# baaivision/Painter

Hardware: AMD Instinct MI355X
Metric: images/sec (896x448 pairs) ViT-L fwd+bwd (higher is better)
Workload: dtype bf16; 1 GPU; painter_vit_large_patch16_input896x448 bf16 batch=8/GPU fwd+bwd on 1xMI355X (BASELINE configs[1]); global_batch=8, image=896x448x3 stitched pair, mode=train (DropPath 0.1), parallelism=dp1, rccl_ranks=0, backend=n/a, grad_allreduce=n/a

## Files before the change

### include/painter_hip.h

```cpp
#ifndef PAINTER_HIP_H
#define PAINTER_HIP_H

#include <stdint.h>

#ifdef __cplusplus
extern "C" {
#endif

#ifndef __HIP__
typedef struct ihipStream_t* hipStream_t;
#endif

enum { PA_F32 = 0, PA_BF16 = 1 };
enum {
    PA_EPI_BIAS = 0,
    PA_EPI_BIAS_F32 = 1,
    PA_EPI_BIAS_GELU = 2,
    PA_EPI_BIAS_RESID = 3
};

#define PA_ABI_VERSION 9
int pa_abi_version(void);
int pa_debug_set(int which, int value);
int pa_debug_get(int which);
// ... 102 lines not shown
int pa_cast_bf16(const float* in, void* out, int64_t n, hipStream_t stream);
int pa_debug_rmw(const float* src, float* scratch, int64_t n, int passes, int nblocks, hipStream_t stream);
int pa_ensemble_resid(const float* x0, const float* a, float* x1, int batch, int group, int L, int D, hipStream_t stream);

int pa_conv3x3_pack(int dtype, const float* w3 , void* w3r , void* wf ,
                    hipStream_t stream);
int pa_decoder_tail_fwd(int dtype, const void* x_nhwc, const void* w3r, const float* b3, const float* ln_gamma,
                        const float* ln_beta, const float* w1 , const float* b1, void* y3 ,
                        float* pred , int batch, int Hi, int Wi, float eps, hipStream_t stream);
int64_t pa_decoder_tail_bwd_workspace_bytes(int batch, int Hi, int Wi);
int pa_decoder_tail_bwd_pointwise(int dtype, const float* dpred, const void* y3, const float* ln_gamma,
                                  const float* ln_beta, const float* w1, void* dy3, float* grads, void* workspace,
                                  int batch, int Hi, int Wi, float eps, hipStream_t stream);
int pa_conv3x3_dgrad_unshuffle(int dtype, const void* dy3, const void* wf, void* dE, int batch, int Hp, int Wp, int P,
                               hipStream_t stream);
int64_t pa_conv3x3_wgrad_workspace_bytes(int batch, int Hi, int Wi);
int pa_conv3x3_wgrad(int dtype, const void* dy3, const void* x_nhwc, float* dw , void* workspace,
                     int batch, int Hi, int Wi, hipStream_t stream);

int pa_live_rows_max(void);
int pa_live_rows(const unsigned char* mask, int mask_batch_stride, int* rowmap, int* live, int* count, int batch, int Hp, int Wp,
                 hipStream_t stream);
int pa_conv3x3_dgrad_unshuffle_live(const void* dy3, const void* wf, void* dE_compact, const int* rowmap, const int* count, int batch,
                                    int Hp, int Wp, int P, hipStream_t stream);
int pa_gather_rows(const void* src, int64_t src_row_bytes, void* dst, int64_t dst_row_bytes, int64_t row_bytes, const int* live,
                   const int* count, int M, hipStream_t stream);
int pa_linear_dgrad_live(const void* dy, int64_t lddy, const void* w, void* dx, int64_t lddx, const int* live, const int* rowmap,
                         const int* count, int M, int N, int K, hipStream_t stream);
int pa_linear_wgrad_live(const void* dy, int64_t lddy, const void* x, int64_t ldx, float* dw, const int* count, int M, int N, int K,
                         hipStream_t stream);
int pa_colsum_live(int dtype, const void* x, int64_t ld, int M, int N, float* out, void* workspace, const int* count, hipStream_t stream);
int pa_fill_dead_rows(void* x, int64_t pitch_bytes, int64_t row_bytes, const int* rowmap, int M, hipStream_t stream);
int pa_decoder_live_ok(int dtype, int batch, int Hp, int Wp, int P, int Kin);

int64_t pa_loss_workspace_bytes(int batch, int Hi, int Wi);
int pa_loss_fwd(const float* pred, const float* tgts, float* valid, const unsigned char* mask, int mask_batch_stride,
                float* out, void* workspace, int batch, int Hi, int Wi, int P, int ignore_rule, float eps_den, int kind,
                float beta, hipStream_t stream);
int pa_loss_bwd(const float* pred, const float* tgts, const float* valid, const unsigned char* mask,
                int mask_batch_stride, const float* dloss, const float* loss_out, float* dpred, int batch, int Hi, int Wi,
                int P, int kind, float beta, hipStream_t stream);
int pa_patchify(const float* img, float* out, int batch, int Hp, int Wp, int P, hipStream_t stream);
int pa_pred_bwd(const float* pred, const float* tgts, const float* valid, const unsigned char* mask, int mask_batch_stride,
                const float* dloss, const float* loss_out, const float* dpatch, float* dpred, float* dpred_loss, int batch, int Hi,
                int Wi, int P, int kind, float beta, hipStream_t stream);

typedef struct PaOptTensor {
    void* p; const void* g; void* m; void* v;
    void* w16;
    int64_t n;
    int32_t group;
    int32_t first_chunk;
} PaOptTensor;
typedef struct PaOptGroups {
    float lr[64], wd[64];
} PaOptGroups;
int pa_opt_chunk_elems(void);
int64_t pa_grad_sumsq_workspace_bytes(int nchunks);
int pa_grad_sumsq(const PaOptTensor* table, int ntensors, int nchunks, float* out2, void* workspace, hipStream_t stream);
int pa_adamw_step(const PaOptTensor* table, int ntensors, int nchunks, const PaOptGroups* groups, double beta1, double beta2,
                  float eps, float* steps, const float* norm_info, const float* grad_scale, const float* found_inf,
                  float max_norm, hipStream_t stream);

int pa_resample_u8(const void* src, int src_h, int src_w, void* dst, int dst_h, int dst_w, int channels, const void* bounds,
                   const void* coeffs, int ksize, int vertical, hipStream_t stream);
int pa_gather_u8(const void* src, int src_h, int src_w, void* dst, int dst_h, int dst_w, int channels, const void* ytab,
// ... 150 lines not shown
```

### painter_amd/csrc/common.h

```cpp
#pragma once
#include <hip/hip_runtime.h>
#include <stdint.h>
#include <cstdlib>

typedef __bf16 bf16;
typedef __attribute__((ext_vector_type(8))) __bf16 bf16x8;
typedef __attribute__((ext_vector_type(16))) float f32x16;

#define DEVI __device__ __forceinline__

template <typename T> struct TT;
template <> struct TT<float> {
    static constexpr int EPC = 4;
    static constexpr int BK = 32;
    static constexpr int KSTEPS = 2;
    static constexpr int SPF = 2;
    typedef uint4 Vec4;
};
template <> struct TT<bf16> {
    static constexpr int EPC = 8;
    static constexpr int BK = 64;
    static constexpr int KSTEPS = 4;
    static constexpr int SPF = 1;
    typedef uint2 Vec4;
// ... 67 lines not shown
    return v;
}

enum Knob {
    KNOB_G256_STAGGER = 0,
    KNOB_G256_NOSTORE = 1,
    KNOB_G256_ORDER = 2,
    KNOB_WGRAD_TARGET = 3,
    KNOB_G256_SHORT_TILES = 4,
    KNOB_G256_ILV = 5,
    KNOB_RELPOS_SPLITS = 6,
    KNOB_ATTN3_FUSE = 7,
    KNOB_ATTN_LIGHT_LAST = 8,
    KNOB_CONV_WGRAD_GROUPS = 9,
    KNOB_LN_BWD_VARIANT = 10,
    KNOB_G256_PATCH = 11,
    KNOB_G256_MIXED = 12,
    KNOB_FREE_13 = 13,
    KNOB_G256_MIXED_NFULL = 14,
    KNOB_FREE_15 = 15,
    KNOB_DROP_SKIP = 16,
    KNOB_DECODER_ROWS = 17,
    KNOB_COUNT = 18
};
inline int g_knob[KNOB_COUNT] = {};
static inline bool drop_skip_on() {
    static const int env = [] { const char* v = getenv("PAINTER_AMD_DROP_SKIP"); return v ? atoi(v) : 1; }();
    return g_knob[KNOB_DROP_SKIP] == 1 ? false : (g_knob[KNOB_DROP_SKIP] == 2 ? true : env != 0);
}
static inline bool decoder_rows_on() {
    static const int env = [] { const char* v = getenv("PAINTER_AMD_DECODER_ROWS"); return v ? atoi(v) : 1; }();
    return g_knob[KNOB_DECODER_ROWS] == 1 ? false : (g_knob[KNOB_DECODER_ROWS] == 2 ? true : env != 0);
}

inline long long g_attn_counts[6] = {0, 0, 0, 0, 0, 0};

DEVI float gelu_f(float x) { return 0.5f * x * (1.0f + erff(x * 0.70710678118654752f)); }
DEVI float gelu_grad_f(float x) {
    const float cdf = 0.5f * (1.0f + erff(x * 0.70710678118654752f));
    const float pdf = 0.39894228040143268f * __expf(-0.5f * x * x);
    return cdf + x * pdf;
}

DEVI void gelu_parts(float x, float& cdf, float& pdf_unnorm) {
    const float z = fabsf(x) * 0.70710678118654752f;
    const float t = __builtin_amdgcn_rcpf(fmaf(0.3275911f, z, 1.0f));
    const float e = __builtin_amdgcn_exp2f(-0.72134752044448170f * x * x);
    float p = fmaf(1.061405429f, t, -1.453152027f);
    p = fmaf(p, t, 1.421413741f);
    p = fmaf(p, t, -0.284496736f);
    p = fmaf(p, t, 0.254829592f);
    const float half_erfc = 0.5f * p * t * e;
    cdf = x >= 0.f ? 1.0f - half_erfc : half_erfc;
    pdf_unnorm = e;
}
DEVI float gelu_fast(float x) {
    float c, e;
    gelu_parts(x, c, e);
    return x * c;
}
typedef __attribute__((ext_vector_type(2))) float f32x2_t;
DEVI void gelu_parts2(f32x2_t x, f32x2_t& cdf, f32x2_t& e) {
    const f32x2_t ax = {fabsf(x[0]), fabsf(x[1])};
    const f32x2_t d = __builtin_elementwise_fma(ax, (f32x2_t){0.23164189f, 0.23164189f}, (f32x2_t){1.0f, 1.0f});
    const f32x2_t t = {__builtin_amdgcn_rcpf(d[0]), __builtin_amdgcn_rcpf(d[1])};
    const f32x2_t xx = x * x * (f32x2_t){-0.72134752044448170f, -0.72134752044448170f};
// ... 53 lines not shown
```

### painter_amd/csrc/elementwise.hip

```cpp
#include "common.h"
#include "../../include/painter_hip.h"

extern "C" int pa_slab_reduce(const float* in, float* out, int64_t n, int nz, int64_t stride, int accumulate, hipStream_t st);

__global__ void cast_bf16_kernel(const float* __restrict__ in, bf16* __restrict__ out, size_t n) {
    size_t i = ((size_t)blockIdx.x * blockDim.x + threadIdx.x) * 4;
    if (i + 4 <= n) {
        const float4 v = *reinterpret_cast<const float4*>(in + i);
        *reinterpret_cast<uint2*>(out + i) = make_uint2(pack_bf16x2(v.x, v.y), pack_bf16x2(v.z, v.w));
    } else {
        for (; i < n; ++i) out[i] = (bf16)in[i];
    }
}
extern "C" int pa_cast_bf16(const float* in, void* out, int64_t n, hipStream_t st) {
    if (n <= 0) return 0;
    PA_LAUNCH(cast_bf16_kernel, dim3((unsigned)((n + 1023) / 1024)), dim3(256), 0, st, in, (bf16*)out, (size_t)n);
    LAUNCH_CHECK();
}

__global__ __launch_bounds__(256) void sparse_rows_kernel(const int* __restrict__ idx, const float* __restrict__ val, int K, const float* __restrict__ x0,
                                                          const float* __restrict__ x1, float* __restrict__ out, int D) {
    __shared__ float red[4][64];
    const int r = blockIdx.y, cl = threadIdx.x & 63, jl = threadIdx.x >> 6, n = blockIdx.x * 64 + cl;
    float acc = 0.f;
// ... 283 lines not shown
        g += dpatch[((size_t)b * L + l) * (size_t)(3 * P * P) + k];
    }
    dpred[idx] = g;
}
extern "C" int pa_pred_bwd(const float* pred, const float* tgts, const float* valid, const unsigned char* mask, int mask_batch_stride,
                           const float* dloss, const float* loss_out, const float* dpatch, float* dpred, float* dpred_loss, int batch, int Hi,
                           int Wi, int P, int kind, float beta, hipStream_t st) {
    if ((dloss == nullptr && dpatch == nullptr) || (dpred_loss != nullptr && dloss == nullptr) || P < 1 || Hi % P || Wi % P)
        return (int)hipErrorInvalidValue;
    const int HW = Hi * Wi;
    PA_LAUNCH(pred_bwd_kernel, dim3((3 * HW + 255) / 256, batch), dim3(256), 0, st, pred, tgts, valid, mask, mask_batch_stride,
              dloss, loss_out, dpatch, dpred, dpred_loss, HW, Wi, P, Wi / P, kind, beta);
    LAUNCH_CHECK();
}

__global__ void patchify_kernel(const float* __restrict__ img, float* __restrict__ out, int Hp, int Wp, int P, size_t n) {
    const size_t i = (size_t)blockIdx.x * blockDim.x + threadIdx.x;
    if (i >= n) return;
    const int PP3 = P * P * 3, L = Hp * Wp;
    const int k = (int)(i % PP3);
    const size_t t = i / PP3;
    const int l = (int)(t % L), b = (int)(t / L);
    const int c = k % 3, q = (k / 3) % P, p = k / (3 * P), h = l / Wp, w = l % Wp;
    out[i] = img[(((size_t)b * 3 + c) * Hp * P + h * P + p) * (size_t)(Wp * P) + w * P + q];
}
extern "C" int pa_patchify(const float* img, float* out, int batch, int Hp, int Wp, int P, hipStream_t st) {
    const size_t n = (size_t)batch * Hp * Wp * P * P * 3;
    PA_LAUNCH(patchify_kernel, dim3((unsigned)((n + 255) / 256)), dim3(256), 0, st, img, out, Hp, Wp, P, n);
    LAUNCH_CHECK();
}

#define TAILP 324
DEVI float oct_sum(float v) { v = quad_sum(v); v += lane_dpp<0x141>(v); return v; }
template <typename T>
__global__ __launch_bounds__(256) void tail_bwd_kernel(const float* __restrict__ dpred, const T* __restrict__ y3, const float* __restrict__ gamma,
                                                       const float* __restrict__ beta, const float* __restrict__ w1, T* __restrict__ dy3,
                                                       float* __restrict__ part, int HW, int npix, float eps) {
    const int lane = threadIdx.x & 63, wave = threadIdx.x >> 6;
    const int sub = lane & 7, slot = (threadIdx.x >> 3);
    const int c0 = sub * 8;
    f32x2_t g2[4], b2[4], w2[3][4];
#pragma unroll
    for (int k = 0; k < 4; ++k) {
        g2[k] = (f32x2_t){gamma[c0 + 2 * k], gamma[c0 + 2 * k + 1]};
        b2[k] = (f32x2_t){beta[c0 + 2 * k], beta[c0 + 2 * k + 1]};
#pragma unroll
        for (int o = 0; o < 3; ++o) w2[o][k] = (f32x2_t){w1[o * 64 + c0 + 2 * k], w1[o * 64 + c0 + 2 * k + 1]};
    }
    const f32x2_t zero2 = {0.f, 0.f};
    f32x2_t ag[4] = {zero2, zero2, zero2, zero2}, ab[4] = {zero2, zero2, zero2, zero2};
    f32x2_t aw[3][4] = {{zero2, zero2, zero2, zero2}, {zero2, zero2, zero2, zero2}, {zero2, zero2, zero2, zero2}};
    float ab1[3] = {0.f, 0.f, 0.f};
    const int stride = gridDim.x * 32;
    struct In { uint4 a, b; float d0, d1, d2; };
    struct Pos { int pix, b, rem; };
    auto advance = [&](Pos& p) {
        p.pix += stride;
        p.rem += stride;
        while (p.rem >= HW) { p.rem -= HW; ++p.b; }
    };
    auto fetch = [&](const Pos& p) {
        In in;
        const int q = min(p.pix, npix - 1);
        const int bb = p.pix < npix ? p.b : (npix - 1) / HW, rr = p.pix < npix ? p.rem : (npix - 1) % HW;
        in.a = *reinterpret_cast<const uint4*>(y3 + (size_t)q * 64 + c0);
        if constexpr (sizeof(T) == 4) in.b = *reinterpret_cast<const uint4*>(y3 + (size_t)q * 64 + c0 + 4);
        else in.b = in.a;
        const float* dp = dpred + (size_t)bb * 3 * HW + rr;
        in.d0 = dp[0]; in.d1 = dp[(size_t)HW]; in.d2 = dp[(size_t)2 * HW];
        return in;
    };
    Pos cur, nxt;
    cur.pix = blockIdx.x * 32 + slot;
    cur.b = cur.pix / HW;
    cur.rem = cur.pix - cur.b * HW;
    nxt = cur;
    In in0 = fetch(nxt);
    advance(nxt);
    In in1 = fetch(nxt);
    advance(nxt);
    for (; cur.pix < npix; advance(cur)) {
        const In in = in0;
        in0 = in1;
        in1 = fetch(nxt);
        advance(nxt);
        const int pix = cur.pix;
        f32x2_t y[4];
        if constexpr (sizeof(T) == 2) {
            const uint4 raw = in.a;
            y[0] = (f32x2_t){bf16_lo(raw.x), bf16_hi(raw.x)}; y[1] = (f32x2_t){bf16_lo(raw.y), bf16_hi(raw.y)};
            y[2] = (f32x2_t){bf16_lo(raw.z), bf16_hi(raw.z)}; y[3] = (f32x2_t){bf16_lo(raw.w), bf16_hi(raw.w)};
        } else {
            y[0] = (f32x2_t){__builtin_bit_cast(float, in.a.x), __builtin_bit_cast(float, in.a.y)};
            y[1] = (f32x2_t){__builtin_bit_cast(float, in.a.z), __builtin_bit_cast(float, in.a.w)};
            y[2] = (f32x2_t){__builtin_bit_cast(float, in.b.x), __builtin_bit_cast(float, in.b.y)};
            y[3] = (f32x2_t){__builtin_bit_cast(float, in.b.z), __builtin_bit_cast(float, in.b.w)};
        }
        const float d0 = in.d0, d1 = in.d1, d2 = in.d2;
        f32x2_t s2 = (y[0] + y[1]) + (y[2] + y[3]);
        const float mu = oct_sum(s2[0] + s2[1]) * (1.f / 64);
        const f32x2_t mu2 = {mu, mu};
        f32x2_t q2 = zero2;
#pragma unroll
        for (int k = 0; k < 4; ++k) { y[k] = y[k] - mu2; q2 = __builtin_elementwise_fma(y[k], y[k], q2); }
        const float rs = 1.f / sqrtf(oct_sum(q2[0] + q2[1]) * (1.f / 64) + eps);
        const f32x2_t rs2 = {rs, rs}, dd0 = {d0, d0}, dd1 = {d1, d1}, dd2 = {d2, d2};
        f32x2_t dxh[4], m1 = zero2, m2 = zero2;
#pragma unroll
        for (int k = 0; k < 4; ++k) {
            const f32x2_t xh = y[k] * rs2;
            const f32x2_t z = __builtin_elementwise_fma(xh, g2[k], b2[k]);
            f32x2_t a, gz;
            if constexpr (sizeof(T) == 2) {
                gelu_both2(z[0], z[1], a, gz);
            } else {
                a = (f32x2_t){gelu_f(z[0]), gelu_f(z[1])};
                gz = (f32x2_t){gelu_grad_f(z[0]), gelu_grad_f(z[1])};
            }
            const f32x2_t da = __builtin_elementwise_fma(dd2, w2[2][k], __builtin_elementwise_fma(dd1, w2[1][k], dd0 * w2[0][k]));
            const f32x2_t dz = da * gz;
            ag[k] = __builtin_elementwise_fma(dz, xh, ag[k]);
            ab[k] = ab[k] + dz;
            aw[0][k] = __builtin_elementwise_fma(dd0, a, aw[0][k]);
            aw[1][k] = __builtin_elementwise_fma(dd1, a, aw[1][k]);
            aw[2][k] = __builtin_elementwise_fma(dd2, a, aw[2][k]);
            dxh[k] = dz * g2[k];
            m1 = m1 + dxh[k];
            m2 = __builtin_elementwise_fma(dxh[k], xh, m2);
            y[k] = xh;
        }
        if (sub == 0) { ab1[0] += d0; ab1[1] += d1; ab1[2] += d2; }
        const float m1s = oct_sum(m1[0] + m1[1]) * (1.f / 64), m2s = oct_sum(m2[0] + m2[1]) * (1.f / 64);
        const f32x2_t mm1 = {m1s, m1s}, nm2 = {-m2s, -m2s};
        f32x2_t r[4];
#pragma unroll
        for (int k = 0; k < 4; ++k) r[k] = rs2 * (__builtin_elementwise_fma(y[k], nm2, dxh[k]) - mm1);
        if constexpr (sizeof(T) == 2) {
            *reinterpret_cast<uint4*>(dy3 + (size_t)pix * 64 + c0) = make_uint4(pack_bf16x2(r[0][0], r[0][1]), pack_bf16x2(r[1][0], r[1][1]),
                                                                                 pack_bf16x2(r[2][0], r[2][1]), pack_bf16x2(r[3][0], r[3][1]));
        } else {
            *reinterpret_cast<float4*>(dy3 + (size_t)pix * 64 + c0) = make_float4(r[0][0], r[0][1], r[1][0], r[1][1]);
            *reinterpret_cast<float4*>(dy3 + (size_t)pix * 64 + c0 + 4) = make_float4(r[2][0], r[2][1], r[3][0], r[3][1]);
        }
    }
    auto wsum = [&](float v) { v += lane_dpp<0x128>(v); v += lane_xor16(v); v += lane_xor32(v); return v; };
    __shared__ float red[4][TAILP];
#pragma unroll
    for (int k = 0; k < 4; ++k)
#pragma unroll
        for (int e = 0; e < 2; ++e) {
            const float vg = wsum(ag[k][e]), vb = wsum(ab[k][e]), v0 = wsum(aw[0][k][e]), v1 = wsum(aw[1][k][e]), v2 = wsum(aw[2][k][e]);
            if (lane < 8) {
                const int c = c0 + 2 * k + e;
                red[wave][c] = vg; red[wave][64 + c] = vb; red[wave][128 + c] = v0; red[wave][192 + c] = v1; red[wave][256 + c] = v2;
            }
        }
    {
        const float t0 = wsum(ab1[0]), t1 = wsum(ab1[1]), t2 = wsum(ab1[2]);
        if (lane == 0) { red[wave][320] = t0; red[wave][321] = t1; red[wave][322] = t2; red[wave][323] = 0.f; }
    }
    __syncthreads();
    for (int i = threadIdx.x; i < TAILP; i += 256) part[(size_t)blockIdx.x * TAILP + i] = (red[0][i] + red[1][i]) + (red[2][i] + red[3][i]);
}
static int tail_bwd_blocks(int npix) {
    int b = (npix + 31) / 32;
    return b > 2048 ? 2048 : b;
}
extern "C" int64_t pa_decoder_tail_bwd_workspace_bytes(int batch, int Hi, int Wi) { return (int64_t)tail_bwd_blocks(batch * Hi * Wi) * TAILP * sizeof(float); }
extern "C" int pa_decoder_tail_bwd_pointwise(int dtype, const float* dpred, const void* y3, const float* ln_gamma, const float* ln_beta,
                                             const float* w1, void* dy3, float* grads, void* workspace, int batch, int Hi, int Wi, float eps,
                                             hipStream_t st) {
    const int npix = batch * Hi * Wi, nb = tail_bwd_blocks(npix);
    float* part = reinterpret_cast<float*>(workspace);
    if (dtype == PA_BF16)
        PA_LAUNCH(tail_bwd_kernel<bf16>, dim3(nb), dim3(256), 0, st, dpred, (const bf16*)y3, ln_gamma, ln_beta, w1, (bf16*)dy3, part, Hi * Wi, npix, eps);
    else
        PA_LAUNCH(tail_bwd_kernel<float>, dim3(nb), dim3(256), 0, st, dpred, (const float*)y3, ln_gamma, ln_beta, w1, (float*)dy3, part, Hi * Wi, npix, eps);
    int e = (int)hipGetLastError();
    if (e) return e;
    return pa_slab_reduce(part, grads, TAILP, nb, TAILP, 0, st);
}

#define LIVE_NT 1024
#define LIVE_MAX_ROWS 49152
__global__ __launch_bounds__(LIVE_NT) void live_rows_kernel(const unsigned char* __restrict__ mask, int mbs, int* __restrict__ rowmap, int* __restrict__ live,
                                                            int* __restrict__ count, int Bn, int Hp, int Wp) {
    __shared__ int sc[2][LIVE_NT];
    extern __shared__ unsigned char flag[];
    const int L = Hp * Wp, n = Bn * L, per = (n + LIVE_NT - 1) / LIVE_NT;
    for (int t = threadIdx.x; t < n; t += LIVE_NT) {
        const int b = t / L, l = t - b * L, i = l / Wp, j = l - i * Wp;
        const unsigned char* m = mask + (size_t)b * mbs;
        unsigned int any = 0;
#pragma unroll
        for (int di = -1; di <= 1; ++di)
#pragma unroll
            for (int dj = -1; dj <= 1; ++dj) {
                const int ii = i + di, jj = j + dj;
                const bool in = ii >= 0 && ii < Hp && jj >= 0 && jj < Wp;
                any |= in ? (unsigned int)m[in ? ii * Wp + jj : 0] : 0u;
            }
        flag[t] = any ? 1 : 0;
    }
    __syncthreads();
    const int t0 = min(n, (int)threadIdx.x * per), t1 = min(n, t0 + per);
    int mine = 0;
    for (int t = t0; t < t1; ++t) mine += flag[t];
    sc[0][threadIdx.x] = mine;
    __syncthreads();
    int cur = 0;
    for (int d = 1; d < LIVE_NT; d <<= 1) {
        const int v = sc[cur][threadIdx.x] + ((int)threadIdx.x >= d ? sc[cur][threadIdx.x - d] : 0);
        sc[cur ^ 1][threadIdx.x] = v;
        cur ^= 1;
        __syncthreads();
    }
    int at = sc[cur][threadIdx.x] - mine;
    for (int t = t0; t < t1; ++t) {
        if (flag[t]) { rowmap[t] = at; live[at] = t; ++at; }
        else rowmap[t] = -1;
    }
    if (threadIdx.x == LIVE_NT - 1) count[0] = sc[cur][LIVE_NT - 1];
}
extern "C" int pa_live_rows_max(void) { return LIVE_MAX_ROWS; }
extern "C" int pa_live_rows(const unsigned char* mask, int mask_batch_stride, int* rowmap, int* live, int* count, int batch, int Hp, int Wp,
                            hipStream_t st) {
    if (batch < 1 || Hp < 1 || Wp < 1 || (int64_t)batch * Hp * Wp > LIVE_MAX_ROWS) return (int)hipErrorInvalidValue;
    const int n = batch * Hp * Wp;
    PA_LAUNCH(live_rows_kernel, dim3(1), dim3(LIVE_NT), (size_t)((n + 15) & ~15), st, mask, mask_batch_stride, rowmap, live, count, batch, Hp, Wp);
    LAUNCH_CHECK();
}
__global__ __launch_bounds__(256) void gather_rows_kernel(const uint4* __restrict__ src, size_t lds16, uint4* __restrict__ dst, size_t ldd16, int row16,
                                                          const int* __restrict__ live, const int* __restrict__ count) {
    const int r = blockIdx.x, cnt = *count;
    if (r >= ((cnt + 127) & ~127)) return;
    if (r < cnt && src == nullptr) return;
    const uint4* s = r < cnt ? src + (size_t)live[r] * lds16 : nullptr;
    uint4* d = dst + (size_t)r * ldd16;
    for (int c = threadIdx.x; c < row16; c += 256) d[c] = s ? s[c] : zero4();
}
extern "C" int pa_gather_rows(const void* src, int64_t src_row_bytes, void* dst, int64_t dst_row_bytes, int64_t row_bytes, const int* live,
                              const int* count, int M, hipStream_t st) {
    if (M < 1 || row_bytes % 16 || src_row_bytes % 16 || dst_row_bytes % 16 || row_bytes > dst_row_bytes || (src != nullptr && row_bytes > src_row_bytes))
        return (int)hipErrorInvalidValue;
    if (((uintptr_t)src | (uintptr_t)dst) & 15) return (int)hipErrorInvalidValue;
    const int Mp = (M + 127) / 128 * 128;
    PA_LAUNCH(gather_rows_kernel, dim3(Mp), dim3(256), 0, st, (const uint4*)src, (size_t)(src_row_bytes / 16), (uint4*)dst, (size_t)(dst_row_bytes / 16),
              (int)(row_bytes / 16), live, count);
    LAUNCH_CHECK();
}
__global__ __launch_bounds__(256) void fill_dead_rows_kernel(uint4* __restrict__ x, size_t pitch16, size_t row16, const int* __restrict__ rowmap) {
    const int r = blockIdx.x;
    if (rowmap[r] >= 0) return;
    uint4* d = x + (size_t)r * pitch16;
    for (size_t c = threadIdx.x; c < row16; c += 256) d[c] = zero4();
}
extern "C" int pa_fill_dead_rows(void* x, int64_t pitch_bytes, int64_t row_bytes, const int* rowmap, int M, hipStream_t st) {
    if (M < 1 || row_bytes % 16 || pitch_bytes % 16 || row_bytes > pitch_bytes || ((uintptr_t)x & 15)) return (int)hipErrorInvalidValue;
    PA_LAUNCH(fill_dead_rows_kernel, dim3(M), dim3(256), 0, st, (uint4*)x, (size_t)(pitch_bytes / 16), (size_t)(row_bytes / 16), rowmap);
    LAUNCH_CHECK();
}

__global__ __launch_bounds__(256) void debug_rmw_kernel(const float* __restrict__ src, float* __restrict__ scratch, size_t n4, int passes) {
    for (int p = 0; p < passes; ++p)
// ... 13 lines not shown
```

### painter_amd/engine.py

```python
import os
from typing import NamedTuple

import torch

from . import hostmath, ops
from ._lib import EPI_BIAS, EPI_BIAS_F32, EPI_BIAS_RESID, KNOB_RELPOS_SPLITS, KNOB_WGRAD_TARGET


_SIDE_STREAM = os.environ.get("PAINTER_AMD_SIDE_STREAM", "1") != "0"
_DBG_SERIAL = os.environ.get("PAINTER_AMD_DEBUG_SERIAL", "0") == "1"
_DBG_TRACE = os.environ.get("PAINTER_AMD_DEBUG_TRACE", "0") == "1"
_configured = False
WGRAD_SIDE_TARGET = 96
RELPOS_SIDE_SPLITS = 8


def _configure_library():
    global _configured
    if _configured:
        return
    from ._lib import lib
    lib.pa_debug_set(KNOB_RELPOS_SPLITS, RELPOS_SIDE_SPLITS if _SIDE_STREAM else 0)
    lib.pa_debug_set(KNOB_WGRAD_TARGET, WGRAD_SIDE_TARGET if _SIDE_STREAM else 0)
    _configured = True
# ... 350 lines not shown
        self.trace = []
        dconcat, dpred_loss = self._backward_decoder(X, dloss, dpatch, want_tgts)
        dx = dyT_next = None
        for i in reversed(range(self.cfg.depth)):
            dx, dyT_next = self._backward_block(X, i, dconcat, dx, dyT_next)
        dimgs, dtgts = self._backward_tokens(X, dx, dpred_loss, want_imgs, want_tgts)
        del dpred_loss
        G = X.G
        if want is not None:
            G = {n: g for n, g in G.items() if g is not None and n in want}
        X.st.join(getattr(self, "tail_probe", None))
        if sync is not None:
            sync.finish()
        if want_imgs or want_tgts:
            return G, dimgs, dtgts
        return G

    def _tr(self, name, t):
        if _DBG_TRACE:
            self.trace.append((name, t.detach().double().abs().sum()))

    def _backward_decoder(self, X, dloss, dpatch, want_tgts):
        c, T, P, S, G, st, need = self.cfg, self.T, X.P, X.S, X.G, X.st, X.need
        B = S.B
        dpred_loss = None
        if dpatch is None:
            dpred = ops.loss_bwd(S.pred, S.tgts, S.valid, S.mask, dloss, S.loss_out, c.P, c.loss_func)
            if want_tgts:
                dpred_loss = dpred
        else:
            dpred, dpred_loss = ops.pred_bwd(S.pred, S.tgts, S.valid, S.mask, dloss, S.loss_out, dpatch, c.P, c.loss_func,
                                             want_loss_term=want_tgts and dloss is not None)
        w1 = P["decoder_pred.3.weight"].reshape(3, c.dec)
        dy3, tg = ops.decoder_tail_bwd_pointwise(dpred, S.y3, P["decoder_pred.1.weight"], P["decoder_pred.1.bias"], w1, 1e-6)
        G["decoder_pred.1.weight"] = tg[0:64]
        G["decoder_pred.1.bias"] = tg[64:128]
        G["decoder_pred.3.weight"] = tg[128:320].reshape(3, c.dec, 1, 1)
        G["decoder_pred.3.bias"] = tg[320:323]
        npix = B * c.H * c.W
        if need("decoder_pred.0.weight") or need("decoder_pred.0.bias"):
            G["decoder_pred.0.weight"], G["decoder_pred.0.bias"] = st.run(
                lambda: (ops.conv3x3_wgrad(dy3, S.E) if need("decoder_pred.0.weight") else None,
                         ops.colsum(dy3.view(npix, c.dec)) if need("decoder_pred.0.bias") else None), dy3, S.E)
        w_de = self.w("decoder_embed.weight", P)
        if dpatch is None and ops.decoder_live_ok(T, B, c.Hp, c.Wp, c.P, w_de.shape[1]):
            rowmap, live, count = ops.live_rows(S.mask, B, c.Hp, c.Wp)
            st.shared(count)
            dE = ops.conv3x3_dgrad_unshuffle_live(dy3, S.wf, rowmap, count, B, c.Hp, c.Wp, c.P)
            del dy3
            X.param_grads("decoder_embed.weight", "decoder_embed.bias", dE, S.concat,
                          wgrad=lambda dy, x: ops.linear_wgrad(dy, x, live=(live, count)),
                          colsum=lambda dy, out=None: ops.colsum_live(dy, count, out=out))
            dconcat = ops.linear_dgrad(dE, w_de, live=(live, rowmap, count))
            if _DBG_TRACE:
                self._tr("dE", dE[:int(count.item())])
        else:
            dE = ops.conv3x3_dgrad_unshuffle(dy3, S.wf, B, c.Hp, c.Wp, c.P)
            del dy3
            X.param_grads("decoder_embed.weight", "decoder_embed.bias", dE, S.concat)
            dconcat = ops.linear_dgrad(dE, w_de)
            self._tr("dE", dE)
        self._tr("dconcat", dconcat)
        del dE
        X.ready(["decoder_embed.weight", "decoder_embed.bias"])
        X.ready([n for n in G if n.startswith("decoder_pred.")])
        return dconcat, dpred_loss

    def block_flat(self, X, i):
        if i not in X.flats:
            D = self.cfg.D
            sizes = [2 * D, 2 * D, 3 * D, D, self.cfg.hidden, D, X.rc_shape[0] * X.rc_shape[1]]
            fb = X.st.shared(torch.empty((sum(sizes),), dtype=torch.float32, device=X.S.imgs.device))
            X.flats[i] = (fb, dict(zip(("n1", "n2", "qkv", "proj", "fc1", "fc2", "rel"), torch.split(fb, sizes))))
        return X.flats[i]

    def _backward_block(self, X, i, dconcat, dx, dyT_next):
        c, T, P, S, G, st, need = self.cfg, self.T, X.P, X.S, X.G, X.st, X.need
        B, L, D = S.B, c.L, c.D
        dev = S.imgs.device
# ... 131 lines not shown
```

### painter_amd/ops.py

```python
import torch

from ._lib import (EPI_BIAS, EPI_BIAS_F32, EPI_BIAS_GELU, EPI_BIAS_RESID, KNOB_DECODER_ROWS, KNOB_DROP_SKIP, PA_BF16, PA_F32, check, lib)

_WS = {}


def stream():
    return torch.cuda.current_stream().cuda_stream


def code(dtype):
    if dtype == torch.bfloat16:
        return PA_BF16
    if dtype == torch.float32:
        return PA_F32
    raise TypeError("painter_amd supports float32 / bfloat16 operand types, got %s" % dtype)


def p(t):
    return 0 if t is None else t.data_ptr()


def workspace(nbytes, device, slot=0):
    key = (device, slot, torch.cuda.current_stream(device).cuda_stream)
# ... 126 lines not shown
    if out is None:
        out = torch.empty((N, K), dtype=torch.float32, device=dy.device)
    ws = workspace(lib.pa_linear_wgrad_workspace_bytes(code(T), M, N, K), dy.device)
    check(lib.pa_linear_wgrad(code(T), p(dy), dy.stride(0), p(x), x.stride(0), p(out), p(ws), M, N, K, stream()),
          "pa_linear_wgrad")
    return out


def colsum(x, out=None):
    M, N = x.shape
    if out is None:
        out = torch.empty((N,), dtype=torch.float32, device=x.device)
    ws = workspace(lib.pa_colsum_workspace_bytes(M, N), x.device)
    check(lib.pa_colsum(code(x.dtype), p(x), x.stride(0), M, N, p(out), p(ws), stream()), "pa_colsum")
    return out


def decoder_rows(mode=None):
    return _knob(KNOB_DECODER_ROWS, mode)


def decoder_live_ok(T, batch, Hp, Wp, P, Kin):
    return T == torch.bfloat16 and bool(lib.pa_decoder_live_ok(code(T), batch, Hp, Wp, P, Kin))


def live_rows(mask_u8, batch, Hp, Wp):
    n = batch * Hp * Wp
    assert mask_u8.dtype in (torch.uint8, torch.bool) and mask_u8.is_cuda and mask_u8.stride(-1) == 1 and mask_u8.shape[-1] == Hp * Wp
    assert mask_u8.shape[0] in (1, batch)
    buf = torch.empty((2 * n + 1,), dtype=torch.int32, device=mask_u8.device)
    rowmap, live, count = buf[:n], buf[n:2 * n], buf[2 * n:]
    check(lib.pa_live_rows(p(mask_u8), _mbs(mask_u8), p(rowmap), p(live), p(count), batch, Hp, Wp, stream()), "pa_live_rows")
    return rowmap, live, count


def padded_rows(n):
    return (n + 127) // 128 * 128


def conv3x3_dgrad_unshuffle_live(dy3, wf, rowmap, count, batch, Hp, Wp, P, out=None):
    assert dy3.dtype == torch.bfloat16
    if out is None:
        out = torch.empty((padded_rows(batch * Hp * Wp), P * P * 64), dtype=dy3.dtype, device=dy3.device)
    assert out.shape == (padded_rows(batch * Hp * Wp), P * P * 64) and out.is_contiguous()
    check(lib.pa_conv3x3_dgrad_unshuffle_live(p(dy3), p(wf), p(out), p(rowmap), p(count), batch, Hp, Wp, P, stream()),
          "pa_conv3x3_dgrad_unshuffle_live")
    return out


def gather_rows(x, live, count, out=None):
    M, N = x.shape
    _req(x)
    if out is None:
        out = torch.empty((padded_rows(M), N), dtype=x.dtype, device=x.device)
    es = x.element_size()
    check(lib.pa_gather_rows(p(x), x.stride(0) * es, p(out), out.stride(0) * es, N * es, p(live), p(count), M, stream()), "pa_gather_rows")
    return out


def linear_wgrad_live(dy, x, count, out=None):
    M, N = dy.shape
    K = x.shape[1]
    _req(dy, torch.bfloat16); _req(x, torch.bfloat16)
    assert x.shape[0] == M and M % 128 == 0
    if out is None:
        out = torch.empty((N, K), dtype=torch.float32, device=dy.device)
# ... 269 lines not shown
    x1 = torch.empty_like(x0)
    check(lib.pa_ensemble_resid(p(x0), p(a), p(x1), batch, group, L, D, stream()), "pa_ensemble_resid")
    return x1


def conv3x3_pack(w3, T):
    w3r = torch.empty((64, 9, 64), dtype=T, device=w3.device)
    wf = torch.empty((64, 9, 64), dtype=T, device=w3.device)
    check(lib.pa_conv3x3_pack(code(T), p(w3), p(w3r), p(wf), stream()), "pa_conv3x3_pack")
    return w3r, wf


def decoder_tail_fwd(x_nhwc, w3r, b3, gamma, beta, w1, b1, eps, save_y3=True):
    B, Hi, Wi, C = x_nhwc.shape
    T = x_nhwc.dtype
    y3 = torch.empty((B, Hi, Wi, C), dtype=T, device=x_nhwc.device) if save_y3 else None
    pred = torch.empty((B, 3, Hi, Wi), dtype=torch.float32, device=x_nhwc.device)
    check(lib.pa_decoder_tail_fwd(code(T), p(x_nhwc), p(w3r), p(b3), p(gamma), p(beta), p(w1), p(b1), p(y3), p(pred), B, Hi, Wi,
                                  float(eps), stream()), "pa_decoder_tail_fwd")
    return pred, y3


def decoder_tail_bwd_pointwise(dpred, y3, gamma, beta, w1, eps):
    B, Hi, Wi, C = y3.shape
    T = y3.dtype
    dy3 = torch.empty_like(y3)
    grads = torch.empty((324,), dtype=torch.float32, device=y3.device)
    ws = workspace(lib.pa_decoder_tail_bwd_workspace_bytes(B, Hi, Wi), y3.device)
    check(lib.pa_decoder_tail_bwd_pointwise(code(T), p(dpred), p(y3), p(gamma), p(beta), p(w1), p(dy3), p(grads), p(ws), B, Hi, Wi,
                                            float(eps), stream()), "pa_decoder_tail_bwd_pointwise")
    return dy3, grads


def conv3x3_dgrad_unshuffle(dy3, wf, batch, Hp, Wp, P):
    T = dy3.dtype
    dE = torch.empty((batch * Hp * Wp, P * P * 64), dtype=T, device=dy3.device)
    check(lib.pa_conv3x3_dgrad_unshuffle(code(T), p(dy3), p(wf), p(dE), batch, Hp, Wp, P, stream()), "pa_conv3x3_dgrad_unshuffle")
    return dE


def conv3x3_wgrad(dy3, x_nhwc):
    B, Hi, Wi, C = x_nhwc.shape
    dw = torch.empty((64, 64, 3, 3), dtype=torch.float32, device=dy3.device)
    ws = workspace(lib.pa_conv3x3_wgrad_workspace_bytes(B, Hi, Wi), dy3.device)
    check(lib.pa_conv3x3_wgrad(code(dy3.dtype), p(dy3), p(x_nhwc), p(dw), p(ws), B, Hi, Wi, stream()), "pa_conv3x3_wgrad")
    return dw


LOSS_KINDS = {"smoothl1": 0, "l1": 1, "l2": 2, "l1l2": 3}


def loss_fwd(pred, tgts, valid, mask_u8, P, ignore_rule, eps_den, kind, beta=0.01):
    B, _, Hi, Wi = pred.shape
    out = torch.empty((2,), dtype=torch.float32, device=pred.device)
    ws = workspace(lib.pa_loss_workspace_bytes(B, Hi, Wi), pred.device)
    check(lib.pa_loss_fwd(p(pred), p(tgts), p(valid), p(mask_u8), _mbs(mask_u8), p(out), p(ws), B, Hi, Wi, P, int(ignore_rule),
                          float(eps_den), LOSS_KINDS[kind], float(beta), stream()), "pa_loss_fwd")
    return out


def loss_bwd(pred, tgts, valid, mask_u8, dloss, loss_out, P, kind, beta=0.01):
    B, _, Hi, Wi = pred.shape
    dpred = torch.empty_like(pred)
    check(lib.pa_loss_bwd(p(pred), p(tgts), p(valid), p(mask_u8), _mbs(mask_u8), p(dloss), p(loss_out), p(dpred), B, Hi, Wi, P,
                          LOSS_KINDS[kind], float(beta), stream()), "pa_loss_bwd")
    return dpred
# ... 19 lines not shown
```

Before: 164.8 images/sec.

## Skip decoder-tail backward work on masked-out patches using per-patch live classes

Adds a live-rows kernel variant that also classifies each patch as masked, neighbour of masked, or dead. The decoder tail pointwise backward uses these classes to skip loads and arithmetic for pixels whose loss gradient is zero, writing zeros to dy3 instead. The engine computes the classes before the tail backward and reuses the resulting rowmap for the later live-row conv dgrad. The cost is an extra per-pixel class lookup in a prefetch pipeline, plus more code complexity around mask semantics.

```diff
diff --git a/include/painter_hip.h b/include/painter_hip.h
--- a/include/painter_hip.h
+++ b/include/painter_hip.h
@@ -158,6 +158,12 @@
 int pa_colsum_live(int dtype, const void* x, int64_t ld, int M, int N, float* out, void* workspace, const int* count, hipStream_t stream);
 int pa_fill_dead_rows(void* x, int64_t pitch_bytes, int64_t row_bytes, const int* rowmap, int M, hipStream_t stream);
 int pa_decoder_live_ok(int dtype, int batch, int Hp, int Wp, int P, int Kin);
+int pa_live_rows_classes(const unsigned char* mask, int mask_batch_stride, int* rowmap, int* live, int* count, int* pcls, int batch, int Hp,
+                         int Wp, hipStream_t stream);
+int pa_decoder_tail_bwd_masked(const float* dpred, const void* y3, const float* ln_gamma, const float* ln_beta, const float* w1, void* dy3,
+                               float* grads, void* workspace, const int* pcls, int batch, int Hi, int Wi, int P, float eps,
+                               hipStream_t stream);
+int pa_decoder_tail_masked_ok(int dtype, int batch, int Hp, int Wp, int P, int Kin);
 
 int64_t pa_loss_workspace_bytes(int batch, int Hi, int Wi);
 int pa_loss_fwd(const float* pred, const float* tgts, float* valid, const unsigned char* mask, int mask_batch_stride,
diff --git a/painter_amd/csrc/common.h b/painter_amd/csrc/common.h
--- a/painter_amd/csrc/common.h
+++ b/painter_amd/csrc/common.h
@@ -123,6 +123,10 @@
     static const int env = [] { const char* v = getenv("PAINTER_AMD_DECODER_ROWS"); return v ? atoi(v) : 1; }();
     return g_knob[KNOB_DECODER_ROWS] == 1 ? false : (g_knob[KNOB_DECODER_ROWS] == 2 ? true : env != 0);
 }
+static inline bool decoder_tail_masked_on() {
+    static const int env = [] { const char* v = getenv("PAINTER_AMD_DECODER_ROWS"); return v ? atoi(v) : 1; }();
+    return decoder_rows_on() && g_knob[KNOB_DECODER_ROWS] != 3 && !(g_knob[KNOB_DECODER_ROWS] == 0 && env == 3);
+}
 
 inline long long g_attn_counts[6] = {0, 0, 0, 0, 0, 0};
 
diff --git a/painter_amd/csrc/elementwise.hip b/painter_amd/csrc/elementwise.hip
--- a/painter_amd/csrc/elementwise.hip
+++ b/painter_amd/csrc/elementwise.hip
@@ -339,10 +339,11 @@
 
 #define TAILP 324
 DEVI float oct_sum(float v) { v = quad_sum(v); v += lane_dpp<0x141>(v); return v; }
-template <typename T>
-__global__ __launch_bounds__(256) void tail_bwd_kernel(const float* __restrict__ dpred, const T* __restrict__ y3, const float* __restrict__ gamma,
-                                                       const float* __restrict__ beta, const float* __restrict__ w1, T* __restrict__ dy3,
-                                                       float* __restrict__ part, int HW, int npix, float eps) {
+typedef __attribute__((address_space(4))) const int cint_k;
+template <typename T, bool CLS>
+DEVI void tail_bwd_body(const float* __restrict__ dpred, const T* __restrict__ y3, const float* __restrict__ gamma,
+                        const float* __restrict__ beta, const float* __restrict__ w1, T* __restrict__ dy3,
+                        float* __restrict__ part, int HW, int npix, float eps, const int* __restrict__ pcls, int Wi, int P) {
     const int lane = threadIdx.x & 63, wave = threadIdx.x >> 6;
     const int sub = lane & 7, slot = (threadIdx.x >> 3);
     const int c0 = sub * 8;
@@ -359,15 +360,31 @@
     f32x2_t aw[3][4] = {{zero2, zero2, zero2, zero2}, {zero2, zero2, zero2, zero2}, {zero2, zero2, zero2, zero2}};
     float ab1[3] = {0.f, 0.f, 0.f};
     const int stride = gridDim.x * 32;
-    struct In { uint4 a, b; float d0, d1, d2; };
+    struct In { uint4 a, b; float d0, d1, d2; int cls; };
     struct Pos { int pix, b, rem; };
     auto advance = [&](Pos& p) {
         p.pix += stride;
         p.rem += stride;
         while (p.rem >= HW) { p.rem -= HW; ++p.b; }
     };
-    auto fetch = [&](const Pos& p) {
+    const int Wp = CLS ? Wi / P : 0, L = CLS ? (HW / Wi / P) * Wp : 0;
+    auto run_class = [&](const Pos& p) -> int {
+        const int wp = __builtin_amdgcn_readfirstlane(p.pix);
+        if (wp >= npix) return 1;
+        const int wb = __builtin_amdgcn_readfirstlane(p.b), wr = __builtin_amdgcn_readfirstlane(p.rem);
+        const int y = wr / Wi, x = wr - y * Wi;
+        return ((cint_k*)pcls)[wb * L + (y / P) * Wp + x / P];
+    };
+    auto fetch = [&](const Pos& p, int cls) {
         In in;
+        in.cls = cls;
+        if constexpr (CLS) {
+            if (cls != 0) {
+                in.a = in.b = zero4();
+                in.d0 = in.d1 = in.d2 = 0.f;
+                return in;
+            }
+        }
         const int q = min(p.pix, npix - 1);
         const int bb = p.pix < npix ? p.b : (npix - 1) / HW, rr = p.pix < npix ? p.rem : (npix - 1) % HW;
         in.a = *reinterpret_cast<const uint4*>(y3 + (size_t)q * 64 + c0);
@@ -382,16 +399,47 @@
     cur.b = cur.pix / HW;
     cur.rem = cur.pix - cur.b * HW;
     nxt = cur;
-    In in0 = fetch(nxt);
-    advance(nxt);
-    In in1 = fetch(nxt);
-    advance(nxt);
+    Pos far = cur;
+    int cls_nxt = 0;
+    In in0, in1;
+    if constexpr (CLS) {
+        const int k0 = run_class(far);
+        advance(far);
+        const int k1 = run_class(far);
+        advance(far);
+        cls_nxt = run_class(far);
+        advance(far);
+        In a = fetch(nxt, k0);
+        advance(nxt);
+        In b = fetch(nxt, k1);
+        advance(nxt);
+        in0 = a; in1 = b;
+    } else {
+        in0 = fetch(nxt, 0);
+        advance(nxt);
+        in1 = fetch(nxt, 0);
+        advance(nxt);
+    }
     for (; cur.pix < npix; advance(cur)) {
         const In in = in0;
         in0 = in1;
-        in1 = fetch(nxt);
+        if constexpr (CLS) {
+            const int cls_far = run_class(far);
+            advance(far);
+            in1 = fetch(nxt, cls_nxt);
+            cls_nxt = cls_far;
+        } else {
+            in1 = fetch(nxt, 0);
+        }
         advance(nxt);
         const int pix = cur.pix;
+        if constexpr (CLS) {
+            if (in.cls != 0) {
+                *reinterpret_cast<uint4*>(dy3 + (size_t)pix * 64 + c0) = zero4();
+                if constexpr (sizeof(T) == 4) *reinterpret_cast<uint4*>(dy3 + (size_t)pix * 64 + c0 + 4) = zero4();
+                continue;
+            }
+        }
         f32x2_t y[4];
         if constexpr (sizeof(T) == 2) {
             const uint4 raw = in.a;
@@ -427,7 +475,9 @@
             const f32x2_t da = __builtin_elementwise_fma(dd2, w2[2][k], __builtin_elementwise_fma(dd1, w2[1][k], dd0 * w2[0][k]));
             const f32x2_t dz = da * gz;
             ag[k] = __builtin_elementwise_fma(dz, xh, ag[k]);
-            ab[k] = ab[k] + dz;
+            f32x2_t dzr = dz;
+            if constexpr (CLS) asm("" : "+v"(dzr));
+            ab[k] = ab[k] + dzr;
             aw[0][k] = __builtin_elementwise_fma(dd0, a, aw[0][k]);
             aw[1][k] = __builtin_elementwise_fma(dd1, a, aw[1][k]);
             aw[2][k] = __builtin_elementwise_fma(dd2, a, aw[2][k]);
@@ -468,6 +518,18 @@
     }
     __syncthreads();
     for (int i = threadIdx.x; i < TAILP; i += 256) part[(size_t)blockIdx.x * TAILP + i] = (red[0][i] + red[1][i]) + (red[2][i] + red[3][i]);
+}
+template <typename T>
+__global__ __launch_bounds__(256) void tail_bwd_kernel(const float* __restrict__ dpred, const T* __restrict__ y3, const float* __restrict__ gamma,
+                                                       const float* __restrict__ beta, const float* __restrict__ w1, T* __restrict__ dy3,
+                                                       float* __restrict__ part, int HW, int npix, float eps) {
+    tail_bwd_body<T, false>(dpred, y3, gamma, beta, w1, dy3, part, HW, npix, eps, nullptr, 0, 0);
+}
+__global__ __launch_bounds__(256) void tail_bwd_masked_kernel(const float* __restrict__ dpred, const bf16* __restrict__ y3, const float* __restrict__ gamma,
+                                                              const float* __restrict__ beta, const float* __restrict__ w1, bf16* __restrict__ dy3,
+                                                              float* __restrict__ part, int HW, int npix, float eps, const int* __restrict__ pcls,
+                                                              int Wi, int P) {
+    tail_bwd_body<bf16, true>(dpred, y3, gamma, beta, w1, dy3, part, HW, npix, eps, pcls, Wi, P);
 }
 static int tail_bwd_blocks(int npix) {
     int b = (npix + 31) / 32;
@@ -487,6 +549,25 @@
     if (e) return e;
     return pa_slab_reduce(part, grads, TAILP, nb, TAILP, 0, st);
 }
+extern "C" int pa_decoder_live_ok(int dtype, int batch, int Hp, int Wp, int P, int Kin);
+extern "C" int pa_decoder_tail_masked_ok(int dtype, int batch, int Hp, int Wp, int P, int Kin) {
+    return pa_decoder_live_ok(dtype, batch, Hp, Wp, P, Kin) && decoder_tail_masked_on() && P >= 8 && P % 8 == 0 &&
+           (int64_t)batch * Hp * Wp * P * P < (int64_t)INT32_MAX - 4 * 2048 * 32;
+}
+extern "C" int pa_decoder_tail_bwd_masked(const float* dpred, const void* y3, const float* ln_gamma, const float* ln_beta, const float* w1,
+                                          void* dy3, float* grads, void* workspace, const int* pcls, int batch, int Hi, int Wi, int P,
+                                          float eps, hipStream_t st) {
+    if (batch < 1 || P < 8 || P % 8 || Hi < P || Wi < P || Hi % P || Wi % P || (int64_t)batch * Hi * Wi >= (int64_t)INT32_MAX - 4 * 2048 * 32 ||
+        ((uintptr_t)pcls & 3))
+        return (int)hipErrorInvalidValue;
+    const int npix = batch * Hi * Wi, nb = tail_bwd_blocks(npix);
+    float* part = reinterpret_cast<float*>(workspace);
+    PA_LAUNCH(tail_bwd_masked_kernel, dim3(nb), dim3(256), 0, st, dpred, (const bf16*)y3, ln_gamma, ln_beta, w1, (bf16*)dy3, part, Hi * Wi, npix, eps,
+              pcls, Wi, P);
+    int e = (int)hipGetLastError();
+    if (e) return e;
+    return pa_slab_reduce(part, grads, TAILP, nb, TAILP, 0, st);
+}
 
 #define LIVE_NT 1024
 #define LIVE_MAX_ROWS 49152
@@ -537,6 +618,81 @@
     PA_LAUNCH(live_rows_kernel, dim3(1), dim3(LIVE_NT), (size_t)((n + 15) & ~15), st, mask, mask_batch_stride, rowmap, live, count, batch, Hp, Wp);
     LAUNCH_CHECK();
 }
+DEVI int live_class(const unsigned char* msk, int t, int L, int Hp, int Wp) {
+    const int b = t / L, l = t - b * L, i = l / Wp, j = l - i * Wp;
+    const unsigned char* m = msk + b * L;
+    unsigned int any = 0;
+#pragma unroll
+    for (int di = -1; di <= 1; ++di)
+#pragma unroll
+        for (int dj = -1; dj <= 1; ++dj) {
+            const int ii = i + di, jj = j + dj;
+            const bool in = ii >= 0 && ii < Hp && jj >= 0 && jj < Wp;
+            any |= in ? (unsigned int)m[in ? ii * Wp + jj : 0] : 0u;
+        }
+    return m[l] ? 0 : (any ? 1 : 2);
+}
+__global__ __launch_bounds__(LIVE_NT) void live_rows_classes_kernel(const unsigned char* __restrict__ mask, int mbs, int* __restrict__ rowmap,
+                                                                    int* __restrict__ live, int* __restrict__ count, int* __restrict__ pcls, int Bn,
+                                                                    int Hp, int Wp) {
+    constexpr int NW = LIVE_NT / 64;
+    __shared__ int wcnt[(LIVE_MAX_ROWS / LIVE_NT) * NW];
+    __shared__ int wtot[NW];
+    extern __shared__ unsigned char msk[];
+    const int tid = threadIdx.x, lane = tid & 63, wave = tid >> 6;
+    const int L = Hp * Wp, n = Bn * L, nchunk = (n + LIVE_NT - 1) / LIVE_NT;
+#pragma unroll 8
+    for (int t = tid; t < n; t += LIVE_NT) {
+        const int b = t / L, l = t - b * L;
+        msk[t] = mask[(size_t)b * mbs + l];
+    }
+    __syncthreads();
+    for (int k = 0; k < nchunk; ++k) {
+        const int t = k * LIVE_NT + tid;
+        const bool lv = t < n && live_class(msk, t, L, Hp, Wp) < 2;
+        const unsigned long long bal = __ballot(lv);
+        if (lane == 0) wcnt[k * NW + wave] = __popcll(bal);
+    }
+    __syncthreads();
+    const int nent = nchunk * NW;
+    const int mine = tid < nent ? wcnt[tid] : 0;
+    int inc = mine;
+#pragma unroll
+    for (int d = 1; d < 64; d <<= 1) {
+        const int up = __shfl_up(inc, d, 64);
+        if (lane >= d) inc += up;
+    }
+    if (lane == 63) wtot[wave] = inc;
+    __syncthreads();
+    int base = 0;
+    for (int w = 0; w < wave; ++w) base += wtot[w];
+    if (tid < nent) wcnt[tid] = base + inc - mine;
+    if (tid == LIVE_NT - 1) count[0] = base + inc;
+    __syncthreads();
+    for (int k = 0; k < nchunk; ++k) {
+        const int t = k * LIVE_NT + tid;
+        const int c = t < n ? live_class(msk, t, L, Hp, Wp) : 2;
+        const unsigned long long bal = __ballot(c < 2);
+        if (t < n) {
+            pcls[t] = c;
+            if (c < 2) {
+                const int at = wcnt[k * NW + wave] + __popcll(bal & ((1ull << lane) - 1));
+                rowmap[t] = at;
+                live[at] = t;
+            } else {
+                rowmap[t] = -1;
+            }
+        }
+    }
+}
+extern "C" int pa_live_rows_classes(const unsigned char* mask, int mask_batch_stride, int* rowmap, int* live, int* count, int* pcls, int batch,
+                                    int Hp, int Wp, hipStream_t st) {
+    if (batch < 1 || Hp < 1 || Wp < 1 || (int64_t)batch * Hp * Wp > LIVE_MAX_ROWS) return (int)hipErrorInvalidValue;
+    const int n = batch * Hp * Wp;
+    PA_LAUNCH(live_rows_classes_kernel, dim3(1), dim3(LIVE_NT), (size_t)((n + 15) & ~15), st, mask, mask_batch_stride, rowmap, live, count, pcls,
+              batch, Hp, Wp);
+    LAUNCH_CHECK();
+}
 __global__ __launch_bounds__(256) void gather_rows_kernel(const uint4* __restrict__ src, size_t lds16, uint4* __restrict__ dst, size_t ldd16, int row16,
                                                           const int* __restrict__ live, const int* __restrict__ count) {
     const int r = blockIdx.x, cnt = *count;
diff --git a/painter_amd/engine.py b/painter_amd/engine.py
--- a/painter_amd/engine.py
+++ b/painter_amd/engine.py
@@ -406,7 +406,14 @@
             dpred, dpred_loss = ops.pred_bwd(S.pred, S.tgts, S.valid, S.mask, dloss, S.loss_out, dpatch, c.P, c.loss_func,
                                              want_loss_term=want_tgts and dloss is not None)
         w1 = P["decoder_pred.3.weight"].reshape(3, c.dec)
-        dy3, tg = ops.decoder_tail_bwd_pointwise(dpred, S.y3, P["decoder_pred.1.weight"], P["decoder_pred.1.bias"], w1, 1e-6)
+        w_de = self.w("decoder_embed.weight", P)
+        live_route = dpatch is None and ops.decoder_live_ok(T, B, c.Hp, c.Wp, c.P, w_de.shape[1])
+        pcls = None
+        if live_route and ops.decoder_tail_masked_ok(T, B, c.Hp, c.Wp, c.P, w_de.shape[1]):
+            rowmap, live, count, pcls = ops.live_rows_classes(S.mask, B, c.Hp, c.Wp)
+            dy3, tg = ops.decoder_tail_bwd_masked(dpred, S.y3, P["decoder_pred.1.weight"], P["decoder_pred.1.bias"], w1, 1e-6, pcls, c.P)
+        else:
+            dy3, tg = ops.decoder_tail_bwd_pointwise(dpred, S.y3, P["decoder_pred.1.weight"], P["decoder_pred.1.bias"], w1, 1e-6)
         G["decoder_pred.1.weight"] = tg[0:64]
         G["decoder_pred.1.bias"] = tg[64:128]
         G["decoder_pred.3.weight"] = tg[128:320].reshape(3, c.dec, 1, 1)
@@ -416,9 +423,9 @@
             G["decoder_pred.0.weight"], G["decoder_pred.0.bias"] = st.run(
                 lambda: (ops.conv3x3_wgrad(dy3, S.E) if need("decoder_pred.0.weight") else None,
                          ops.colsum(dy3.view(npix, c.dec)) if need("decoder_pred.0.bias") else None), dy3, S.E)
-        w_de = self.w("decoder_embed.weight", P)
-        if dpatch is None and ops.decoder_live_ok(T, B, c.Hp, c.Wp, c.P, w_de.shape[1]):
-            rowmap, live, count = ops.live_rows(S.mask, B, c.Hp, c.Wp)
+        if live_route:
+            if pcls is None:
+                rowmap, live, count = ops.live_rows(S.mask, B, c.Hp, c.Wp)
             st.shared(count)
             dE = ops.conv3x3_dgrad_unshuffle_live(dy3, S.wf, rowmap, count, B, c.Hp, c.Wp, c.P)
             del dy3
diff --git a/painter_amd/ops.py b/painter_amd/ops.py
--- a/painter_amd/ops.py
+++ b/painter_amd/ops.py
@@ -182,6 +182,21 @@
     rowmap, live, count = buf[:n], buf[n:2 * n], buf[2 * n:]
     check(lib.pa_live_rows(p(mask_u8), _mbs(mask_u8), p(rowmap), p(live), p(count), batch, Hp, Wp, stream()), "pa_live_rows")
     return rowmap, live, count
+
+
+def decoder_tail_masked_ok(T, batch, Hp, Wp, P, Kin):
+    return T == torch.bfloat16 and bool(lib.pa_decoder_tail_masked_ok(code(T), batch, Hp, Wp, P, Kin))
+
+
+def live_rows_classes(mask_u8, batch, Hp, Wp):
+    n = batch * Hp * Wp
+    assert mask_u8.dtype in (torch.uint8, torch.bool) and mask_u8.is_cuda and mask_u8.stride(-1) == 1 and mask_u8.shape[-1] == Hp * Wp
+    assert mask_u8.shape[0] in (1, batch)
+    buf = torch.empty((3 * n + 1,), dtype=torch.int32, device=mask_u8.device)
+    pcls, rowmap, live, count = buf[:n], buf[n:2 * n], buf[2 * n:3 * n], buf[3 * n:]
+    check(lib.pa_live_rows_classes(p(mask_u8), _mbs(mask_u8), p(rowmap), p(live), p(count), p(pcls), batch, Hp, Wp, stream()),
+          "pa_live_rows_classes")
+    return rowmap, live, count, pcls
 
 
 def padded_rows(n):
@@ -517,6 +532,18 @@
     return dy3, grads
 
 
+def decoder_tail_bwd_masked(dpred, y3, gamma, beta, w1, eps, pcls, P):
+    B, Hi, Wi, C = y3.shape
+    _req(y3, torch.bfloat16); _req(pcls, torch.int32)
+    assert y3.is_contiguous() and C == 64 and pcls.numel() == B * (Hi // P) * (Wi // P)
+    dy3 = torch.empty_like(y3)
+    grads = torch.empty((324,), dtype=torch.float32, device=y3.device)
+    ws = workspace(lib.pa_decoder_tail_bwd_workspace_bytes(B, Hi, Wi), y3.device)
+    check(lib.pa_decoder_tail_bwd_masked(p(dpred), p(y3), p(gamma), p(beta), p(w1), p(dy3), p(grads), p(ws), p(pcls), B, Hi, Wi, P,
+                                         float(eps), stream()), "pa_decoder_tail_bwd_masked")
+    return dy3, grads
+
+
 def conv3x3_dgrad_unshuffle(dy3, wf, batch, Hp, Wp, P):
     T = dy3.dtype
     dE = torch.empty((batch * Hp * Wp, P * P * 64), dtype=T, device=dy3.device)
```

Result: no change. 164.7 images/sec (median of 2 runs) (-0.0%).
